# oxylusengine/Oxylus

Hardware: NVIDIA H100
Metric: meshlet_instances_culled_per_s (higher is better)
Workload: dtype f32

## Files before the change

oxylus_b200/csrc/kernels_tri.cuh:

```cuda
#pragma once
#include <climits>

#include "oxc_exact.cuh"
#include "oxc_raster_core.cuh"
#include "oxc_tma.cuh"

namespace oxc {

#ifndef OXC_TRI_THREADS
#define OXC_TRI_THREADS 256
#endif
constexpr int TRI_THREADS = OXC_TRI_THREADS;
constexpr int TRI_WARPS = TRI_THREADS / 32;

struct TriParams {
  const OxcMeshletInstance* meshlet_instances;
  const InstCull* inst;
  const InstGeom* geom;
  const OxcMeshletInstanceVisibility* vis;
  const OxcDispatchIndirectCommand* tri_cmd;
  const uint32_t* visible_indices;
  const uint32_t* id_base;
  uint32_t late;
  uint32_t* reordered_indices;
// ... 74 lines not shown
  const uint32_t id_base = p.id_base ? __ldg(p.id_base) : 0u;
  const uint32_t n_tiles = (count + TRI_WARPS - 1) / TRI_WARPS;
  float4* clip_s = clip_all[warp];
  for (uint32_t tile = blockIdx.x; tile < n_tiles; tile += gridDim.x) {
    const uint32_t g = tile * TRI_WARPS + warp;
    bool pass[2] = {false, false};
    uint32_t rank[2] = {0, 0}, wtotal = 0, data_id = 0;
    if (g < count) {
      const MeshletWork w = load_meshlet(p, first + g, id_base, clip_s, lane);
      data_id = w.data_id;
#pragma unroll
      for (int k = 0; k < 2; k++) {
        const uint32_t t = lane + 32u * k;
        float4 c0, c1, c2;
        pass[k] = t < w.tri_count && triangle_passes(w, t, clip_s, c0, c1, c2);
        if (pass[k] && p.small_primitive_cull && tri_covers_no_sample(c0, c1, c2, p.f_width, p.f_height, p.width, p.height)) pass[k] = false;
        const uint32_t bal = __ballot_sync(0xffffffffu, pass[k]);
        rank[k] = wtotal + __popc(bal & ((1u << lane) - 1u));
        wtotal += __popc(bal);
      }
      __syncwarp();
    }
    if (lane == 0) warp_cnt[warp] = wtotal;
    __syncthreads();
    if (threadIdx.x == 0) {
      uint32_t s = 0;
#pragma unroll
      for (int k = 0; k < TRI_WARPS; k++) { const uint32_t c = warp_cnt[k]; warp_cnt[k] = s; s += c; }
      base_s = s ? atomicAdd(&p.draw_cmd->index_count, s * 3u) : 0u;
    }
    __syncthreads();
    const uint32_t wbase = base_s + warp_cnt[warp] * 3u;
#pragma unroll
    for (int k = 0; k < 2; k++)
      if (pass[k]) {
        const uint32_t t = lane + 32u * k, off = wbase + rank[k] * 3u, masked = data_id << OXC_VIS_PRIMITIVE_BITS;
        p.reordered_indices[off + 0] = masked | ((t * 3u + 0u) & OXC_VIS_PRIMITIVE_MASK);
        p.reordered_indices[off + 1] = masked | ((t * 3u + 1u) & OXC_VIS_PRIMITIVE_MASK);
        p.reordered_indices[off + 2] = masked | ((t * 3u + 2u) & OXC_VIS_PRIMITIVE_MASK);
      }
    __syncthreads();
  }
}

#ifndef OXC_RASTER_MIN_BLOCKS
#define OXC_RASTER_MIN_BLOCKS 3
#endif
#ifndef OXC_RASTER_BIG_PIXELS
#define OXC_RASTER_BIG_PIXELS 32
#endif
#ifndef OXC_RASTER_BATCH
#define OXC_RASTER_BATCH 8
#endif
constexpr int MICRO_STAGE_BYTES = 224;
constexpr int RASTER_BATCH = OXC_RASTER_BATCH;
static_assert(RASTER_BATCH >= 1 && RASTER_BATCH <= 32, "one header per lane: a grab holds at most 32 meshlets");
constexpr int RASTER_BIG_PIXELS = OXC_RASTER_BIG_PIXELS;

struct MeshletHeader {
  uint32_t gid, inst, vertex_offset, vertex_count, tri_offset, tri_count;
  const uint32_t* micro;
  const uint32_t* vidx;
  const uint2* pos;
};

OXC_DI MeshletHeader fetch_header(const TriParams& p, uint32_t slot, uint32_t id_base) {
  MeshletHeader h;
  h.gid = __ldg(&p.visible_indices[slot]);
  const uint2 mi = __ldg(reinterpret_cast<const uint2*>(p.meshlet_instances) + (h.gid - id_base));
  const InstGeom* g = p.geom + mi.x;
  const uint4 g0 = __ldg(reinterpret_cast<const uint4*>(g));
  const uint4 g1 = __ldg(reinterpret_cast<const uint4*>(g) + 1);
  const OxcMeshlet* meshlets = reinterpret_cast<const OxcMeshlet*>(((uint64_t)g0.y << 32) | g0.x);
  const uint4 m = __ldg(reinterpret_cast<const uint4*>(meshlets + mi.y));
  h.inst = mi.x;
  h.vertex_offset = m.x;
  h.tri_offset = m.y;
  h.vertex_count = min(m.z, (uint32_t)OXC_MESHLET_MAX_VERTICES);
  h.tri_count = min(m.w, (uint32_t)OXC_MESHLET_MAX_PRIMITIVES);
  h.micro = reinterpret_cast<const uint32_t*>(((uint64_t)g0.w << 32) | g0.z);
  h.vidx = reinterpret_cast<const uint32_t*>(((uint64_t)g1.y << 32) | g1.x) + m.x;
  h.pos = reinterpret_cast<const uint2*>(((uint64_t)g1.w << 32) | g1.z);
  return h;
}

OXC_DI MeshletHeader bcast_header(const MeshletHeader& h, int src) {
  MeshletHeader o;
  o.gid = __shfl_sync(0xffffffffu, h.gid, src); o.inst = __shfl_sync(0xffffffffu, h.inst, src);
  o.vertex_offset = 0;
  o.vertex_count = __shfl_sync(0xffffffffu, h.vertex_count, src);
  o.tri_offset = __shfl_sync(0xffffffffu, h.tri_offset, src); o.tri_count = __shfl_sync(0xffffffffu, h.tri_count, src);
  o.micro = reinterpret_cast<const uint32_t*>(__shfl_sync(0xffffffffu, reinterpret_cast<unsigned long long>(h.micro), src));
  o.vidx = reinterpret_cast<const uint32_t*>(__shfl_sync(0xffffffffu, reinterpret_cast<unsigned long long>(h.vidx), src));
  o.pos = reinterpret_cast<const uint2*>(__shfl_sync(0xffffffffu, reinterpret_cast<unsigned long long>(h.pos), src));
  return o;
}

constexpr int BIG_CHUNK_W = 64, BIG_CHUNK_H = 32;

OXC_DI void big_entry_store(uint4* dst, const TriSetup& s, int px0, int px1, int py0, int py1, uint32_t data) {
  dst[0] = make_uint4((uint32_t)s.ax, (uint32_t)s.ay, (uint32_t)s.bx, (uint32_t)s.by);
  dst[1] = make_uint4((uint32_t)s.cx, (uint32_t)s.cy, __float_as_uint(s.za), __float_as_uint(s.dzb));
  dst[2] = make_uint4(__float_as_uint(s.dzc), (uint32_t)px0, (uint32_t)px1, (uint32_t)py0);
  dst[3] = make_uint4((uint32_t)py1, (uint32_t)s.bias, data, 0u);
}

OXC_DI void big_entry_load(const uint4* src, TriSetup& s, uint32_t& data) {
  const uint4 a = src[0], b = src[1], c = src[2], d = src[3];
  s.ax = (int)a.x; s.ay = (int)a.y; s.bx = (int)a.z; s.by = (int)a.w;
  s.cx = (int)b.x; s.cy = (int)b.y; s.za = __uint_as_float(b.z); s.dzb = __uint_as_float(b.w);
// ... 11 lines not shown
  if (base + n > p.big_capacity) {
    for (uint32_t k = base; k < p.big_capacity; k++) big_entry_store(p.big_queue + (size_t)k * 4, s, 1, 0, 1, 0, data);
    return false;
  }
  uint32_t k = base;
  for (uint32_t cy = 0; cy < ch; cy++)
    for (uint32_t cx = 0; cx < cw; cx++, k++) {
      const int x0 = s.px0 + (int)(cx * BIG_CHUNK_W), y0 = s.py0 + (int)(cy * BIG_CHUNK_H);
      big_entry_store(p.big_queue + (size_t)k * 4, s, x0, min(s.px1, x0 + BIG_CHUNK_W - 1), y0, min(s.py1, y0 + BIG_CHUNK_H - 1), data);
    }
  return true;
}

constexpr uint32_t BIG_PUSH_ALONE = 4;
OXC_DI uint32_t big_chunk_count(const TriSetup& s) {
  return ((uint32_t)(s.px1 - s.px0) / BIG_CHUNK_W + 1u) * ((uint32_t)(s.py1 - s.py0) / BIG_CHUNK_H + 1u);
}

OXC_DI bool big_push_warp(const TriParams& p, const TriSetup& s, uint32_t data, uint32_t lane) {
  const uint32_t cw = (uint32_t)(s.px1 - s.px0) / BIG_CHUNK_W + 1u, ch = (uint32_t)(s.py1 - s.py0) / BIG_CHUNK_H + 1u;
  const uint32_t n = cw * ch;
  uint32_t base = 0xFFFFFFFFu;
  if (lane == 0 && *reinterpret_cast<volatile uint32_t*>(&p.big_counters[0]) < p.big_capacity) base = atomicAdd(&p.big_counters[0], n);
  base = __shfl_sync(0xffffffffu, base, 0);
  if (base >= p.big_capacity) return false;
  if (base + n > p.big_capacity) {
    for (uint32_t k = base + lane; k < p.big_capacity; k += 32) big_entry_store(p.big_queue + (size_t)k * 4, s, 1, 0, 1, 0, data);
    return false;
  }
  for (uint32_t k = lane; k < n; k += 32) {
    const uint32_t cy = k / cw, cx = k - cy * cw;
    const int x0 = s.px0 + (int)(cx * BIG_CHUNK_W), y0 = s.py0 + (int)(cy * BIG_CHUNK_H);
    big_entry_store(p.big_queue + (size_t)(base + k) * 4, s, x0, min(s.px1, x0 + BIG_CHUNK_W - 1), y0, min(s.py1, y0 + BIG_CHUNK_H - 1), data);
  }
  return true;
}

__global__ void __launch_bounds__(256) k_raster_big(const __grid_constant__ TriParams p) {
  const uint32_t lane = threadIdx.x & 31;
  const uint32_t total = min(p.big_counters[0], p.big_capacity);
  const int lx = lane & 7, ly = lane >> 3;
  for (uint32_t i = blockIdx.x * (blockDim.x >> 5) + (threadIdx.x >> 5); i < total; i += gridDim.x * (blockDim.x >> 5)) {
    TriSetup b;
    uint32_t data;
    big_entry_load(p.big_queue + (size_t)i * 4, b, data);
    for (int ty = b.py0; ty <= b.py1; ty += 4)
      for (int tx = b.px0; tx <= b.px1; tx += 8) {
        const int px = tx + lx, py = ty + ly;
        if (px <= b.px1 && py <= b.py1) raster_pixel(b, px, py, data, p.visbuf, p.width);
      }
  }
}

template <bool PREFETCH_GRAB>
__global__ void __launch_bounds__(TRI_THREADS, OXC_RASTER_MIN_BLOCKS) k_raster_visbuffer(const __grid_constant__ TriParams p) {
  __shared__ float4 clip_all[TRI_WARPS][OXC_MESHLET_MAX_VERTICES];
  __shared__ ScreenVert scr_all[TRI_WARPS][OXC_MESHLET_MAX_VERTICES];
  const uint32_t lane = threadIdx.x & 31, warp = threadIdx.x >> 5;
#ifndef OXC_RASTER_NO_SMEM_MICRO
#define OXC_RASTER_SMEM_MICRO 1
#endif
#ifdef OXC_RASTER_SMEM_MICRO
  __shared__ uint32_t micro_w[TRI_WARPS][52];
#endif
#ifdef OXC_RASTER_TMA_MICRO
  __shared__ __align__(16) uint8_t micro_all[TRI_WARPS][MICRO_STAGE_BYTES];
  __shared__ __align__(8) uint64_t micro_bar[TRI_WARPS];
  if (lane == 0) { mbar_init(&micro_bar[warp], 1); mbar_fence_init(); }
  __syncwarp();
  uint32_t micro_phase = 0;
#endif
  const uint32_t first = p.late ? p.vis->early_visible_meshlet_instances : 0u;
  const uint32_t count = p.tri_cmd->x;
  const uint32_t id_base = p.id_base ? __ldg(p.id_base) : 0u;
  float4* clip_s = clip_all[warp];
  ScreenVert* scr_s = scr_all[warp];
  uint32_t kept = 0;
#ifdef OXC_RASTER_STATS
  unsigned long long t_entry, t_chase = 0, t_proc = 0, n_done = 0, n_grabs = 0;
  asm volatile("mov.u64 %0, %%globaltimer;" : "=l"(t_entry));
#endif
  const uint32_t n_warps2 = gridDim.x * TRI_WARPS * 2u;
  uint32_t g_next = 0, batch_next = 1;
  if (PREFETCH_GRAB && lane == 0) {
    batch_next = min((uint32_t)RASTER_BATCH, max(1u, count / n_warps2));
    g_next = atomicAdd(p.work_counter, batch_next);
  }
  for (;;) {
    uint32_t g0 = 0, batch = 1;
    if (PREFETCH_GRAB) {
      g0 = __shfl_sync(0xffffffffu, g_next, 0);
      batch = __shfl_sync(0xffffffffu, batch_next, 0);
      if (g0 >= count) break;
      if (lane == 0) {
        const uint32_t seen = g0 + batch;
        const uint32_t rem = count > seen ? count - seen : 0u;
        batch_next = min((uint32_t)RASTER_BATCH, max(1u, rem / n_warps2));
        g_next = atomicAdd(p.work_counter, batch_next);
      }
    } else {
      if (lane == 0) {
        const uint32_t seen = *reinterpret_cast<volatile uint32_t*>(p.work_counter);
        const uint32_t rem = count > seen ? count - seen : 0u;
        batch = min((uint32_t)RASTER_BATCH, max(1u, rem / n_warps2));
        g0 = atomicAdd(p.work_counter, batch);
      }
      g0 = __shfl_sync(0xffffffffu, g0, 0);
      batch = __shfl_sync(0xffffffffu, batch, 0);
      if (g0 >= count) break;
    }
    const uint32_t nb = min(batch, count - g0);
    const uint32_t my_survivor = g0 + lane;
#ifdef OXC_RASTER_STATS
    unsigned long long t_a, t_b, t_c;
    asm volatile("mov.u64 %0, %%globaltimer;" : "=l"(t_a));
#endif
    MeshletHeader mine;
    mine.gid = 0; mine.inst = 0; mine.vertex_offset = 0; mine.vertex_count = 0; mine.tri_offset = 0; mine.tri_count = 0;
    mine.micro = nullptr; mine.vidx = nullptr; mine.pos = nullptr;
    if (lane < nb) mine = fetch_header(p, first + my_survivor, id_base);
    MeshletHeader cur = bcast_header(mine, 0);
    uint32_t vi0 = lane < cur.vertex_count ? __ldg(&cur.vidx[lane]) : 0u;
    uint32_t vi1 = lane + 32u < cur.vertex_count ? __ldg(&cur.vidx[lane + 32u]) : 0u;
#ifdef OXC_RASTER_STATS
    if (vi0 + vi1 == 0xFFFFFFFFu) kept++;
    asm volatile("mov.u64 %0, %%globaltimer;" : "=l"(t_b));
#endif
    for (uint32_t j = 0; j < nb; j++) {
      const MeshletHeader w = cur;
#ifdef OXC_RASTER_TMA_MICRO
      const uint64_t micro_addr = reinterpret_cast<uint64_t>(w.micro) + w.tri_offset;
      const uint32_t micro_skew = (uint32_t)(micro_addr & 15u);
      if (lane == 0) {
        const uint32_t bytes = (micro_skew + w.tri_count * 3u + 15u) & ~15u;
        mbar_expect_tx(&micro_bar[warp], bytes);
        tma_load_1d(micro_all[warp], reinterpret_cast<const void*>(micro_addr - micro_skew), bytes, &micro_bar[warp]);
      }
#endif
#ifdef OXC_RASTER_SMEM_MICRO
      {
        const uint32_t n_words = ((w.tri_offset & 3u) + w.tri_count * 3u + 3u) >> 2;
        const uint32_t* src = w.micro + (w.tri_offset >> 2);
        const uint32_t m0 = lane < n_words ? __ldg(src + lane) : 0u;
        const uint32_t m1 = lane + 32u < n_words ? __ldg(src + lane + 32u) : 0u;
        micro_w[warp][lane] = m0;
        if (lane < 20) micro_w[warp][lane + 32] = m1;
      }
#endif
      const uint2 q0 = lane < w.vertex_count ? __ldg(&w.pos[vi0]) : make_uint2(0, 0);
      const uint2 q1 = lane + 32u < w.vertex_count ? __ldg(&w.pos[vi1]) : make_uint2(0, 0);
      if (j + 1 < nb) {
        cur = bcast_header(mine, (int)(j + 1));
        vi0 = lane < cur.vertex_count ? __ldg(&cur.vidx[lane]) : 0u;
        vi1 = lane + 32u < cur.vertex_count ? __ldg(&cur.vidx[lane + 32u]) : 0u;
      }
      const InstCull* ic = p.inst + w.inst;
      const float4 r0 = __ldg(&ic->mvp_row[0]), r1 = __ldg(&ic->mvp_row[1]), r2 = __ldg(&ic->mvp_row[2]), r3 = __ldg(&ic->mvp_row[3]);
      {
        const float x = dequantize_half_hw(q0.x & 0xFFFFu), y = dequantize_half_hw(q0.x >> 16), z = dequantize_half_hw(q0.y & 0xFFFFu);
        const float4 c = make_float4(row_dot_p1(r0, x, y, z), row_dot_p1(r1, x, y, z), row_dot_p1(r2, x, y, z), row_dot_p1(r3, x, y, z));
        clip_s[lane] = c;
        scr_s[lane] = to_screen(c, p.f_width, p.f_height);
      }
      if (w.vertex_count > 32u) {
        const float x = dequantize_half_hw(q1.x & 0xFFFFu), y = dequantize_half_hw(q1.x >> 16), z = dequantize_half_hw(q1.y & 0xFFFFu);
        const float4 c = make_float4(row_dot_p1(r0, x, y, z), row_dot_p1(r1, x, y, z), row_dot_p1(r2, x, y, z), row_dot_p1(r3, x, y, z));
        clip_s[lane + 32] = c;
        scr_s[lane + 32] = to_screen(c, p.f_width, p.f_height);
      }
      __syncwarp();
#ifdef OXC_RASTER_TMA_MICRO
      mbar_wait(&micro_bar[warp], micro_phase);
      micro_phase ^= 1u;
      const uint8_t* micro_s = micro_all[warp] + micro_skew;
#endif
      const uint32_t rounds = (w.tri_count + 31u) >> 5;
      for (uint32_t k = 0; k < rounds; k++) {
        const uint32_t t = lane + 32u * k;
        bool pass = false;
        TriSetup s;
        bool draw = false;
        if (t < w.tri_count) {
#ifdef OXC_RASTER_TMA_MICRO
          const uint32_t i0 = micro_s[t * 3u + 0u], i1 = micro_s[t * 3u + 1u], i2 = micro_s[t * 3u + 2u];
#elif defined(OXC_RASTER_SMEM_MICRO)
          const uint8_t* mb = reinterpret_cast<const uint8_t*>(micro_w[warp]) + (w.tri_offset & 3u) + t * 3u;
          const uint32_t i0 = mb[0], i1 = mb[1], i2 = mb[2];
#else
          const uint32_t base = w.tri_offset + t * 3u;
          const uint32_t i0 = micro_index(w.micro, base + 0u), i1 = micro_index(w.micro, base + 1u), i2 = micro_index(w.micro, base + 2u);
#endif
          if (max(i0, max(i1, i2)) < w.vertex_count) {
            const float4 c0 = clip_s[i0], c1 = clip_s[i1], c2 = clip_s[i2];
            pass = c0.z >= 0.0f && c1.z >= 0.0f && c2.z >= 0.0f && !triangle_backface(c0, c1, c2);
            if (pass) {
              const int why = tri_setup(scr_s[i0], scr_s[i1], scr_s[i2], p.width, p.height, s);
              draw = why == TRI_DRAW;
              if (why == TRI_NO_SAMPLE && p.small_primitive_cull) pass = false;
              if (why == TRI_INVALID_VERTEX && p.clip_queue) {
                const uint32_t slot = atomicAdd(p.clip_counter, 1u);
                if (slot < p.clip_capacity) p.clip_queue[slot] = (w.gid << p.prim_bits) | t;
                else atomicOr(p.status, (uint32_t)OXC_STATUS_CLIP_OVERFLOW);
              }
            }
          }
        }
        kept += pass ? 1u : 0u;
        const uint32_t data = (w.gid << p.prim_bits) | t;
        const int bw = draw ? s.px1 - s.px0 + 1 : 0, bh = draw ? s.py1 - s.py0 + 1 : 0;
#if defined(OXC_RASTER_STATS) && OXC_RASTER_STATS == 1
        {
          const int area = (draw && bw * bh <= RASTER_BIG_PIXELS) ? bw * bh : 0;
          const int mx = __reduce_max_sync(0xffffffffu, area), sm = __reduce_add_sync(0xffffffffu, area);
          const int nd = __popc(__ballot_sync(0xffffffffu, area > 0));
          const int nbig = __popc(__ballot_sync(0xffffffffu, draw && bw * bh > RASTER_BIG_PIXELS));
          if (lane == 0) {
            unsigned long long* st = reinterpret_cast<unsigned long long*>(p.big_queue) + (size_t)p.big_capacity * 8 + (p.late ? 64 : 0);
            atomicAdd(&st[min(mx, 33)], 1ull);
            atomicAdd(&st[40], (unsigned long long)sm);
            atomicAdd(&st[41], (unsigned long long)mx);
            atomicAdd(&st[42], (unsigned long long)nd);
            atomicAdd(&st[43], 1ull);
            atomicAdd(&st[44], (unsigned long long)nbig);
          }
        }
#endif
        bool big = draw && (bw * bh > RASTER_BIG_PIXELS);
        if (draw && !big) raster_small(s, data, p.visbuf, p.width);
        const bool few = big && big_chunk_count(s) <= BIG_PUSH_ALONE;
// ... 138 lines not shown
```

oxylus_b200/csrc/oxc_raster_core.cuh:

```cuda
#pragma once
#include <climits>

#include "oxc_exact.cuh"

namespace oxc {

struct __align__(16) ScreenVert {
  int fx, fy;
  float z;
  int pad;
};

OXC_DI ScreenVert to_screen(float4 c, float fW, float fH) {
  ScreenVert v;
  v.fx = INT_MIN; v.fy = 0; v.z = 0.f; v.pad = 0;
  if (!(c.w > 0.0f)) return v;
  const float rw = fd(1.0f, c.w);
  const float nx = fm(c.x, rw), ny = fm(c.y, rw);
  const float sx = fm(fa(fm(nx, 0.5f), 0.5f), fW), sy = fm(fa(fm(ny, 0.5f), 0.5f), fH);
  const float qx = floorf(fa(fm(sx, 256.0f), 0.5f)), qy = floorf(fa(fm(sy, 256.0f), 0.5f));
  if (!(fabsf(qx) <= 4194304.0f && fabsf(qy) <= 4194304.0f)) return v;
  v.fx = (int)qx; v.fy = (int)qy; v.z = fm(c.z, rw);
  return v;
}
// ... 31 lines not shown
  const int miny = min(v0.fy, min(v1.fy, v2.fy)), maxy = max(v0.fy, max(v1.fy, v2.fy));
  s.px0 = max(0, (minx - 128 + 255) >> 8);
  s.px1 = min((int)W - 1, (maxx - 128) >> 8);
  s.py0 = max(0, (miny - 128 + 255) >> 8);
  s.py1 = min((int)H - 1, (maxy - 128) >> 8);
  if (s.px1 < s.px0 || s.py1 < s.py0) return TRI_NO_SAMPLE;
  s.narrow = (maxx - minx) < 16384 && (maxy - miny) < 16384;
  long long area2;
  if (s.narrow) area2 = (long long)((v1.fx - v0.fx) * (v2.fy - v0.fy) - (v1.fy - v0.fy) * (v2.fx - v0.fx));
  else area2 = orient2d(v0.fx, v0.fy, v1.fx, v1.fy, v2.fx, v2.fy);
  if (area2 >= 0) return TRI_BACK_OR_DEGENERATE;
  s.ax = v0.fx; s.ay = v0.fy; s.bx = v2.fx; s.by = v2.fy; s.cx = v1.fx; s.cy = v1.fy;
  const float fa_ = (float)(-area2);
  s.za = v0.z;
  s.dzb = fd(fs(v2.z, v0.z), fa_);
  s.dzc = fd(fs(v1.z, v0.z), fa_);
  s.bias = edge_bias_bit(s.bx, s.by, s.cx, s.cy) | (edge_bias_bit(s.cx, s.cy, s.ax, s.ay) << 1) |
           (edge_bias_bit(s.ax, s.ay, s.bx, s.by) << 2);
  return TRI_DRAW;
}

OXC_DI void shade_pixel(const TriSetup& s, long long e0, long long e1, long long e2, int px, int py, uint32_t data,
                        unsigned long long* vis, uint32_t W) {
  if ((e0 - (s.bias & 1)) < 0 || (e1 - ((s.bias >> 1) & 1)) < 0 || (e2 - ((s.bias >> 2) & 1)) < 0) return;
  const float zz = fa(fa(s.za, fm((float)e1, s.dzb)), fm((float)e2, s.dzc));
  if (!(zz >= 0.0f && zz <= 1.0f)) return;
  uint32_t zb = __float_as_uint(zz);
  zb = zb == 0x80000000u ? 0u : zb;
  const unsigned long long v = ((unsigned long long)zb << 32) | data;
  unsigned long long* ptr = vis + (size_t)py * W + px;
  atomicMax(ptr, v);
}

OXC_DI void raster_pixel(const TriSetup& s, int px, int py, uint32_t data, unsigned long long* vis, uint32_t W) {
  const int sx = px * 256 + 128, sy = py * 256 + 128;
  shade_pixel(s, orient2d(s.bx, s.by, s.cx, s.cy, sx, sy), orient2d(s.cx, s.cy, s.ax, s.ay, sx, sy),
              orient2d(s.ax, s.ay, s.bx, s.by, sx, sy), px, py, data, vis, W);
}

OXC_DI int orient2d_32(int ax, int ay, int bx, int by, int cx, int cy) { return (bx - ax) * (cy - ay) - (by - ay) * (cx - ax); }

OXC_DI void shade_pixel_32(const TriSetup& s, int e0, int e1, int e2, int px, int py, uint32_t data, unsigned long long* vis,
                           uint32_t W) {
  if ((e0 - (s.bias & 1)) < 0 || (e1 - ((s.bias >> 1) & 1)) < 0 || (e2 - ((s.bias >> 2) & 1)) < 0) return;
  const float zz = fa(fa(s.za, fm((float)e1, s.dzb)), fm((float)e2, s.dzc));
  if (!(zz >= 0.0f && zz <= 1.0f)) return;
  uint32_t zb = __float_as_uint(zz);
  zb = zb == 0x80000000u ? 0u : zb;
  const unsigned long long v = ((unsigned long long)zb << 32) | data;
  unsigned long long* ptr = vis + (size_t)py * W + px;
  atomicMax(ptr, v);
}

OXC_DI void raster_small(const TriSetup& s, uint32_t data, unsigned long long* vis, uint32_t W) {
  const int sx0 = s.px0 * 256 + 128, sy0 = s.py0 * 256 + 128;
  if (s.narrow) {
    int r0 = orient2d_32(s.bx, s.by, s.cx, s.cy, sx0, sy0), r1 = orient2d_32(s.cx, s.cy, s.ax, s.ay, sx0, sy0),
        r2 = orient2d_32(s.ax, s.ay, s.bx, s.by, sx0, sy0);
    const int dx0 = -(s.cy - s.by) * 256, dy0 = (s.cx - s.bx) * 256, dx1 = -(s.ay - s.cy) * 256, dy1 = (s.ax - s.cx) * 256,
              dx2 = -(s.by - s.ay) * 256, dy2 = (s.bx - s.ax) * 256;
    for (int py = s.py0; py <= s.py1; py++) {
      int e0 = r0, e1 = r1, e2 = r2;
      for (int px = s.px0; px <= s.px1; px++) {
        shade_pixel_32(s, e0, e1, e2, px, py, data, vis, W);
        e0 += dx0; e1 += dx1; e2 += dx2;
      }
      r0 += dy0; r1 += dy1; r2 += dy2;
    }
    return;
  }
  long long r0 = orient2d(s.bx, s.by, s.cx, s.cy, sx0, sy0);
  long long r1 = orient2d(s.cx, s.cy, s.ax, s.ay, sx0, sy0);
  long long r2 = orient2d(s.ax, s.ay, s.bx, s.by, sx0, sy0);
  const long long dx0 = -(long long)(s.cy - s.by) * 256, dy0 = (long long)(s.cx - s.bx) * 256;
  const long long dx1 = -(long long)(s.ay - s.cy) * 256, dy1 = (long long)(s.ax - s.cx) * 256;
  const long long dx2 = -(long long)(s.by - s.ay) * 256, dy2 = (long long)(s.bx - s.ax) * 256;
  for (int py = s.py0; py <= s.py1; py++) {
    long long e0 = r0, e1 = r1, e2 = r2;
    for (int px = s.px0; px <= s.px1; px++) {
      shade_pixel(s, e0, e1, e2, px, py, data, vis, W);
      e0 += dx0; e1 += dx1; e2 += dx2;
    }
    r0 += dy0; r1 += dy1; r2 += dy2;
  }
}

OXC_DI float clip_plane_distance(const float4 v, int plane) {
  switch (plane) {
    case 0: return fs(v.w, v.z);
    case 1: return fa(v.w, v.x);
    case 2: return fs(v.w, v.x);
    case 3: return fa(v.w, v.y);
    default: return fs(v.w, v.y);
  }
}

OXC_DI int clip_polygon(float4 c0, float4 c1, float4 c2, float4 (*poly)[12], int& cur) {
  int n = 3;
  cur = 0;
  poly[0][0] = c0; poly[0][1] = c1; poly[0][2] = c2;
  for (int plane = 0; plane < 5 && n >= 3; plane++) {
    const float4* in = poly[cur];
    float4* out = poly[cur ^ 1];
    int m = 0;
    for (int i = 0; i < n; i++) {
      const float4 A = in[i], B = in[(i + 1) % n];
// ... 19 lines not shown
```

oxylus_b200/csrc/oxcull.cu:

```cuda
#include <cuda_runtime.h>

#include <atomic>
#include <cstdarg>
#include <cstdio>
#include <cstdlib>
#include <cstring>
#include <new>
#include <vector>

#include <dlfcn.h>
#include <nccl.h>

#include "kernels_cull.cuh"
#include "kernels_decode.cuh"
#include "kernels_hiz.cuh"
#include "kernels_mgpu.cuh"
#include "kernels_tri.cuh"
#include "kernels_alpha.cuh"

using namespace oxc;

namespace {

thread_local char g_err[512] = "";
// ... 261 lines not shown
  TRY(dalloc(&c->d_clip_queue, (size_t)c->clip_capacity));
  c->d_clip_counter = c->d_raster_work + 3;
  TRY(dalloc(&c->d_id_base_auto, 1));
  TRY(dalloc(&c->d_status, 1));
  c->prim_bits = info->wide_ids ? OXC_VIS_WIDE_PRIMITIVE_BITS : OXC_VIS_PRIMITIVE_BITS;
  if (info->alloc_reordered_indices) TRY(dalloc(&c->d_reordered, (size_t)N * OXC_MESHLET_MAX_PRIMITIVES * 3));
  if (info->max_views > 1) {
    TRY(dalloc(&c->d_view_planes, (size_t)I * info->max_views));
    TRY(dalloc(&c->d_view_bits, (size_t)N));
    TRY(dalloc(&c->d_view_counts, (size_t)OXC_MAX_VIEWS));
    TRY(dalloc(&c->d_inst_views, (size_t)I * info->max_views));
  }
  {
    uint32_t m = info->hiz_width > info->hiz_height ? info->hiz_width : info->hiz_height, levels = 0;
    while (m) { levels++; m >>= 1; }
    levels = levels < OXC_HIZ_MAX_LEVELS ? levels : OXC_HIZ_MAX_LEVELS;
    uint32_t off = 0;
    for (uint32_t l = 0; l < OXC_HIZ_MAX_LEVELS; l++) {
      c->hiz.level_offset[l] = off;
      if (l < levels) {
        uint32_t mw = info->hiz_width >> l, mh = info->hiz_height >> l;
        off += (mw < 1 ? 1 : mw) * (mh < 1 ? 1 : mh);
      }
    }
    c->hiz.width = info->hiz_width; c->hiz.height = info->hiz_height; c->hiz.levels = levels;
    c->hiz_total = off;
    TRY(dalloc(&c->d_hiz, (size_t)off));
    c->hiz.data = c->d_hiz;
  }
#undef TRY
  CK(cudaMemset(c->d_mask, 0, (size_t)c->mask_words * 4));
  CK(cudaMemset(c->d_hiz, 0, (size_t)c->hiz_total * 4));
  CK(cudaMemset(c->d_vis, 0, sizeof(OxcMeshletInstanceVisibility)));
  CK(cudaMemset(c->d_tri_counter, 0, 8));
  CK(cudaMemset(c->d_status, 0, 4));
  OxcDispatchIndirectCommand one{0, 1, 1};
  CK(cudaMemcpy(c->d_cull_meshlets_cmd, &one, sizeof one, cudaMemcpyHostToDevice));
  CK(cudaMemcpy(c->d_cull_triangles_cmd, &one, sizeof one, cudaMemcpyHostToDevice));
  OxcDrawIndexedIndirectCommand dc{0, 1, 0, 0, 0};
  CK(cudaMemcpy(c->d_draw_cmd, &dc, sizeof dc, cudaMemcpyHostToDevice));
#define OCC(dst, kern, threads) CK(cudaOccupancyMaxActiveBlocksPerMultiprocessor(&(dst), kern, threads, 0))
#define OCCC(dst, H, O, L)                                                                                                        \
  CK(cudaFuncSetAttribute(k_cull_meshlets<H, O, L, false>, cudaFuncAttributeMaxDynamicSharedMemorySize, (int)sizeof(CullShared<O && !L>)));  \
  CK(cudaFuncSetAttribute(k_cull_meshlets<H, O, L, true>, cudaFuncAttributeMaxDynamicSharedMemorySize, (int)sizeof(CullShared<O && !L>)));   \
  CK(cudaOccupancyMaxActiveBlocksPerMultiprocessor(&(dst), (k_cull_meshlets<H, O, L, false>), CULL_THREADS, sizeof(CullShared<O && !L>)))
  OCCC(c->occ_cull[0][0][0], false, false, false);
  OCCC(c->occ_cull[1][0][0], true, false, false);
  OCCC(c->occ_cull[1][0][1], true, false, true);
  OCCC(c->occ_cull[1][1][0], true, true, false);
  OCCC(c->occ_cull[1][1][1], true, true, true);
#undef OCCC
  c->occ_cull[0][0][1] = c->occ_cull[0][1][0] = c->occ_cull[0][1][1] = c->occ_cull[0][0][0];
  OCC(c->occ_tri, k_cull_triangles, TRI_THREADS);
  OCC(c->occ_raster, k_raster_visbuffer<false>, TRI_THREADS);
  OCC(c->occ_mv, k_cull_meshlets_multiview, CULL_THREADS);
#undef OCC
  *out_ctx = c;
  return OXC_OK;
}

void oxc_destroy(OxcContext* c) {
  if (!c) return;
  cudaSetDevice(c->device);
  if (c->mg.active) { cudaDeviceSynchronize(); mgpu_release(c); }
  cudaFree(c->d_meshes); cudaFree(c->d_mesh_instances); cudaFree(c->d_transforms); cudaFree(c->d_blob);
  cudaFree(c->d_lod_aabb); cudaFree(c->d_inst); cudaFree(c->d_geom); cudaFree(c->d_counts); cudaFree(c->d_block_sums);
  cudaFree(c->d_meshlet_instances); cudaFree(c->d_slabs); cudaFree(c->d_visible); cudaFree(c->d_mask); cudaFree(c->d_vis);
  cudaFree(c->d_cull_meshlets_cmd); cudaFree(c->d_cull_triangles_cmd); cudaFree(c->d_draw_cmd);
  cudaFree(c->d_reordered); cudaFree(c->d_tri_counter); cudaFree(c->d_raster_work); cudaFree(c->d_big_queue); cudaFree(c->d_clip_queue); cudaFree(c->d_id_base_auto); cudaFree(c->d_status); cudaFree(c->d_hiz);
  cudaFree(c->d_view_planes); cudaFree(c->d_view_bits); cudaFree(c->d_view_counts); cudaFree(c->d_inst_views);
  cudaFree(c->d_alpha_materials); cudaFree(c->d_alpha_lists); cudaFree(c->d_alpha_cmd);
  delete c;
}

int oxc_set_scene(OxcContext* c, const OxcSceneDesc* sc, void* stream) {
  if (!c || !sc) return fail(OXC_E_INVALID, "null argument");
  cudaStream_t s = static_cast<cudaStream_t>(stream);
  CK(cudaSetDevice(c->device));
  if (sc->mesh_instance_count > c->info.max_mesh_instances)
    return fail(OXC_E_CAPACITY, "mesh_instance_count %u > max_mesh_instances %u", sc->mesh_instance_count, c->info.max_mesh_instances);
  if (sc->mesh_count == 0 || !sc->meshes || !sc->blob || !sc->transforms || (sc->mesh_instance_count && !sc->mesh_instances))
    return fail(OXC_E_INVALID, "scene tables missing");
  struct Reloc { uint64_t lod_record, src, size; int field; };
  std::vector<Reloc> relocs;
  uint64_t reloc_bytes = 0;
  for (uint32_t m = 0; m < sc->mesh_count; m++) {
    const OxcMesh& me = sc->meshes[m];
    if (me.lod_count == 0 || me.lod_count > OXC_MESH_MAX_LODS) return fail(OXC_E_INVALID, "mesh %u: lod_count %u not in 1..%d", m, me.lod_count, OXC_MESH_MAX_LODS);
    if ((me.vertex_positions & 7u) || (me.vertex_normals & 3u) || (me.texture_coords & 3u) || (me.lods & 7u))
      return fail(OXC_E_INVALID, "mesh %u: vertex_positions / lods need 8-byte, normals / texcoords 4-byte aligned blob offsets", m);
    if (me.lods + (uint64_t)me.lod_count * sizeof(OxcMeshLOD) > sc->blob_size || me.vertex_positions + (uint64_t)me.vertex_count * 8u > sc->blob_size)
      return fail(OXC_E_INVALID, "mesh %u: offsets outside the blob", m);
    const OxcMeshLOD* lods = reinterpret_cast<const OxcMeshLOD*>(sc->blob + me.lods);
    for (uint32_t l = 0; l < me.lod_count; l++) {
      OxcMeshLOD d;
      memcpy(&d, &lods[l], sizeof d);
      if ((d.meshlets & 7u) || (d.meshlet_bounds & 7u) || (d.local_triangle_indices & 3u) || (d.indirect_vertex_indices & 3u))
        return fail(OXC_E_INVALID, "mesh %u lod %u: meshlets / meshlet_bounds need 8-byte, index arrays 4-byte aligned blob offsets", m, l);
      if (d.meshlets + (uint64_t)d.meshlet_count * sizeof(OxcMeshlet) > sc->blob_size ||
          d.meshlet_bounds + (uint64_t)d.meshlet_count * sizeof(OxcMeshletBounds) > sc->blob_size ||
          d.local_triangle_indices + (uint64_t)d.local_triangle_indices_count > sc->blob_size ||
          d.indirect_vertex_indices + (uint64_t)d.indirect_vertex_indices_count * 4u > sc->blob_size)
        return fail(OXC_E_INVALID, "mesh %u lod %u: arrays outside the blob", m, l);
      const uint64_t rec = me.lods + (uint64_t)l * sizeof(OxcMeshLOD);
      if (d.meshlets & 15u) { relocs.push_back({rec, d.meshlets, (uint64_t)d.meshlet_count * sizeof(OxcMeshlet), 0}); reloc_bytes += (relocs.back().size + 15u) & ~15ull; }
      if (d.meshlet_bounds & 15u) { relocs.push_back({rec, d.meshlet_bounds, (uint64_t)d.meshlet_count * sizeof(OxcMeshletBounds), 1}); reloc_bytes += (relocs.back().size + 15u) & ~15ull; }
    }
// ... 285 lines not shown
  uint32_t grid = (uint32_t)(c->sm_count * (c->occ_tri > 0 ? c->occ_tri : 1));
  if (grid > tiles) grid = tiles;
  if (grid == 0) grid = 1;
  k_cull_triangles<<<grid, TRI_THREADS, 0, s>>>(p);
  LAUNCHED();
  return OXC_OK;
}

int oxc_clear_visbuffer(OxcContext* c, uint64_t* vis, uint32_t w, uint32_t h, void* stream) {
  if (!c || !vis) return fail(OXC_E_INVALID, "null argument");
  cudaStream_t s = static_cast<cudaStream_t>(stream);
  CK(cudaSetDevice(c->device));
  const size_t n = (size_t)w * h;
  k_clear_visbuffer<<<c->sm_count * 8, 256, 0, s>>>(reinterpret_cast<unsigned long long*>(vis), n);
  LAUNCHED();
  CK(cudaMemsetAsync(c->d_tri_counter, 0, 8, s));
  return OXC_OK;
}

int oxc_raster_visbuffer(OxcContext* c, const OxcCullCamera* cam, uint32_t flags, uint32_t w, uint32_t h, uint64_t* vis,
                         int small_primitive_cull, void* stream) {
  if (!c || !cam || !vis) return fail(OXC_E_INVALID, "null argument");
  if (c->scene_id_bound > (1ull << (32u - c->prim_bits)))
    return fail(OXC_E_CAPACITY, "the scene can emit %llu meshlet instances: ids overflow the %u id bits of the vis-buffer word (visbuffer.slang:9-10)%s",
                (unsigned long long)c->scene_id_bound, 32u - c->prim_bits, c->info.wide_ids ? "" : "; create the context with wide_ids = 1 (26 + 6 bit packing)");
  cudaStream_t s = static_cast<cudaStream_t>(stream);
  CK(cudaSetDevice(c->device));
  TriParams p{};
  int rc = tri_common(c, cam, flags, s, &p);
  if (rc != OXC_OK) return rc;
  p.visbuf = reinterpret_cast<unsigned long long*>(vis); p.width = w; p.height = h; p.f_width = (float)w; p.f_height = (float)h;
  p.small_primitive_cull = small_primitive_cull ? 1u : 0u;
  p.work_counter = c->d_raster_work;
  CK(cudaMemsetAsync(c->d_raster_work, 0, 16, s));
  uint32_t tiles = (c->info.max_meshlet_instances + TRI_WARPS - 1) / TRI_WARPS;
  uint32_t grid = (uint32_t)(c->sm_count * (c->occ_raster > 0 ? c->occ_raster : 1));
  if (grid > tiles) grid = tiles;
  if (grid == 0) grid = 1;
  p.big_queue = c->d_big_queue; p.big_counters = c->d_big_counters; p.big_capacity = c->big_capacity;
  p.clip_queue = c->d_clip_queue; p.clip_counter = c->d_clip_counter; p.clip_capacity = c->clip_capacity;
  TriParams pm = p;
  AlphaParams ap{};
  if (c->alpha_active) {
    ap.mesh_instances = c->d_mesh_instances; ap.materials = c->d_alpha_materials; ap.material_count = c->alpha_material_count;
    ap.opaque_list = c->d_alpha_lists; ap.masked_list = c->d_alpha_lists + c->info.max_meshlet_instances;
    ap.opaque_cmd = reinterpret_cast<OxcDispatchIndirectCommand*>(c->d_alpha_cmd);
    ap.masked_cmd = reinterpret_cast<OxcDispatchIndirectCommand*>(c->d_alpha_cmd + 16);
    CK(cudaMemsetAsync(c->d_alpha_cmd, 0, 64, s));
    k_partition_alpha<<<c->sm_count * 4, 256, 0, s>>>(p, ap);
    LAUNCHED();
    pm.visible_indices = ap.opaque_list; pm.tri_cmd = ap.opaque_cmd;
    pm.vis = reinterpret_cast<const OxcMeshletInstanceVisibility*>(c->d_alpha_cmd + 32);
  }
  if (p.late) k_raster_visbuffer<true><<<grid, TRI_THREADS, 0, s>>>(pm);
  else k_raster_visbuffer<false><<<grid, TRI_THREADS, 0, s>>>(pm);
  LAUNCHED();
  k_raster_clip_queue<<<c->sm_count, 128, 0, s>>>(p);
  LAUNCHED();
  if (c->alpha_active) {
    k_raster_alpha<false><<<c->sm_count * 8, ALPHA_THREADS, 0, s>>>(p, ap);
    LAUNCHED();
  }
  k_raster_big<<<c->sm_count * 8, 256, 0, s>>>(p);
  LAUNCHED();
  return OXC_OK;
}

int oxc_raster_overdraw(OxcContext* c, const OxcCullCamera* cam, uint32_t flags, uint32_t w, uint32_t h, uint32_t* overdraw, int after_frame,
                        void* stream) {
  if (!c || !cam || !overdraw) return fail(OXC_E_INVALID, "null argument");
  cudaStream_t s = static_cast<cudaStream_t>(stream);
  CK(cudaSetDevice(c->device));
  TriParams p{};
  int rc = tri_common(c, cam, flags, s, &p);
  if (rc != OXC_OK) return rc;
  p.width = w; p.height = h; p.f_width = (float)w; p.f_height = (float)h;
  AlphaParams ap{};
  ap.mesh_instances = c->d_mesh_instances; ap.overdraw = overdraw; ap.count_from_visibility = after_frame ? 1u : 0u;
  if (c->alpha_active) { ap.materials = c->d_alpha_materials; ap.material_count = c->alpha_material_count; }
  k_raster_alpha<true><<<c->sm_count * 8, ALPHA_THREADS, 0, s>>>(p, ap);
  LAUNCHED();
  return OXC_OK;
}

int oxc_clear_overdraw(OxcContext* c, uint32_t* overdraw, uint32_t w, uint32_t h, void* stream) {
  if (!c || !overdraw) return fail(OXC_E_INVALID, "null argument");
  CK(cudaSetDevice(c->device));
  CK(cudaMemsetAsync(overdraw, 0, (size_t)w * h * 4, static_cast<cudaStream_t>(stream)));
  return OXC_OK;
}

static float host_dequantize_half(uint16_t h) {
  const uint32_t sgn = ((uint32_t)h & 0x8000u) << 16, em = (uint32_t)h & 0x7fffu;
  uint32_t r = (em + (112u << 10)) << 13;
  r = (em < (1u << 10)) ? 0u : r;
  r += (em >= (31u << 10)) ? (112u << 23) : 0u;
  const uint32_t bits = sgn | r;
  float f;
  memcpy(&f, &bits, 4);
  return f;
}

int oxc_set_materials(OxcContext* c, const OxcMaterialTable* t, void* stream) {
  if (!c) return fail(OXC_E_INVALID, "null context");
  cudaStream_t s = static_cast<cudaStream_t>(stream);
  CK(cudaSetDevice(c->device));
  if (!t || t->material_count == 0) {
    c->alpha_active = false;
// ... 678 lines not shown
```

Measured before the change: 1.807 billion.

## Always prefetch raster work grabs; add opt-in meshlet sample classification path

Drops the PREFETCH_GRAB template so every raster launch, including the early pass, issues the next atomic work grab one iteration ahead instead of reading the counter and grabbing synchronously. It also adds a compile-time CLASSIFY path, off by default. That path computes a meshlet screen bounding box with warp reductions, skips rasterizing meshlets that cover no pixel centre, and handles meshlets covering only a few samples in sample-major order with warp max reductions and a single atomicMax per pixel. The prefetch is meant to hide atomic latency in the early pass, at the cost of always holding one grab in flight.

New measurement: 2.035 billion, median of 6. +12.6%, better.

```diff
diff --git a/oxylus_b200/csrc/kernels_tri.cuh b/oxylus_b200/csrc/kernels_tri.cuh
--- a/oxylus_b200/csrc/kernels_tri.cuh
+++ b/oxylus_b200/csrc/kernels_tri.cuh
@@ -150,10 +150,21 @@
 #ifndef OXC_RASTER_BATCH
 #define OXC_RASTER_BATCH 8
 #endif
+#ifndef OXC_RASTER_CLASSIFY
+#define OXC_RASTER_CLASSIFY 0
+#endif
+#ifndef OXC_RASTER_SAMPLE_MAJOR
+#define OXC_RASTER_SAMPLE_MAJOR 4
+#endif
 constexpr int MICRO_STAGE_BYTES = 224;
 constexpr int RASTER_BATCH = OXC_RASTER_BATCH;
 static_assert(RASTER_BATCH >= 1 && RASTER_BATCH <= 32, "one header per lane: a grab holds at most 32 meshlets");
 constexpr int RASTER_BIG_PIXELS = OXC_RASTER_BIG_PIXELS;
+constexpr int RASTER_SAMPLE_MAJOR = OXC_RASTER_SAMPLE_MAJOR;
+static_assert(RASTER_SAMPLE_MAJOR >= 0 && RASTER_SAMPLE_MAJOR <= 32 && RASTER_SAMPLE_MAJOR <= RASTER_BIG_PIXELS, "sample-major limit");
+
+OXC_DI uint32_t bias_s32(int x) { return (uint32_t)x ^ 0x80000000u; }
+OXC_DI int unbias_s32(uint32_t x) { return (int)(x ^ 0x80000000u); }
 
 struct MeshletHeader {
   uint32_t gid, inst, vertex_offset, vertex_count, tri_offset, tri_count;
@@ -271,7 +282,6 @@
   }
 }
 
-template <bool PREFETCH_GRAB>
 __global__ void __launch_bounds__(TRI_THREADS, OXC_RASTER_MIN_BLOCKS) k_raster_visbuffer(const __grid_constant__ TriParams p) {
   __shared__ float4 clip_all[TRI_WARPS][OXC_MESHLET_MAX_VERTICES];
   __shared__ ScreenVert scr_all[TRI_WARPS][OXC_MESHLET_MAX_VERTICES];
@@ -301,32 +311,18 @@
 #endif
   const uint32_t n_warps2 = gridDim.x * TRI_WARPS * 2u;
   uint32_t g_next = 0, batch_next = 1;
-  if (PREFETCH_GRAB && lane == 0) {
+  if (lane == 0) {
     batch_next = min((uint32_t)RASTER_BATCH, max(1u, count / n_warps2));
     g_next = atomicAdd(p.work_counter, batch_next);
   }
   for (;;) {
-    uint32_t g0 = 0, batch = 1;
-    if (PREFETCH_GRAB) {
-      g0 = __shfl_sync(0xffffffffu, g_next, 0);
-      batch = __shfl_sync(0xffffffffu, batch_next, 0);
-      if (g0 >= count) break;
-      if (lane == 0) {
-        const uint32_t seen = g0 + batch;
-        const uint32_t rem = count > seen ? count - seen : 0u;
-        batch_next = min((uint32_t)RASTER_BATCH, max(1u, rem / n_warps2));
-        g_next = atomicAdd(p.work_counter, batch_next);
-      }
-    } else {
-      if (lane == 0) {
-        const uint32_t seen = *reinterpret_cast<volatile uint32_t*>(p.work_counter);
-        const uint32_t rem = count > seen ? count - seen : 0u;
-        batch = min((uint32_t)RASTER_BATCH, max(1u, rem / n_warps2));
-        g0 = atomicAdd(p.work_counter, batch);
-      }
-      g0 = __shfl_sync(0xffffffffu, g0, 0);
-      batch = __shfl_sync(0xffffffffu, batch, 0);
-      if (g0 >= count) break;
+    const uint32_t g0 = __shfl_sync(0xffffffffu, g_next, 0), batch = __shfl_sync(0xffffffffu, batch_next, 0);
+    if (g0 >= count) break;
+    if (lane == 0) {
+      const uint32_t seen = g0 + batch;
+      const uint32_t rem = count > seen ? count - seen : 0u;
+      batch_next = min((uint32_t)RASTER_BATCH, max(1u, rem / n_warps2));
+      g_next = atomicAdd(p.work_counter, batch_next);
     }
     const uint32_t nb = min(batch, count - g0);
     const uint32_t my_survivor = g0 + lane;
@@ -375,17 +371,35 @@
       }
       const InstCull* ic = p.inst + w.inst;
       const float4 r0 = __ldg(&ic->mvp_row[0]), r1 = __ldg(&ic->mvp_row[1]), r2 = __ldg(&ic->mvp_row[2]), r3 = __ldg(&ic->mvp_row[3]);
+#if OXC_RASTER_CLASSIFY
+      uint32_t bx0 = bias_s32(1 << 23), by0 = bias_s32(1 << 23), bx1 = bias_s32(-(1 << 23)), by1 = bias_s32(-(1 << 23));
+      bool bad = false;
+#endif
       {
         const float x = dequantize_half_hw(q0.x & 0xFFFFu), y = dequantize_half_hw(q0.x >> 16), z = dequantize_half_hw(q0.y & 0xFFFFu);
         const float4 c = make_float4(row_dot_p1(r0, x, y, z), row_dot_p1(r1, x, y, z), row_dot_p1(r2, x, y, z), row_dot_p1(r3, x, y, z));
         clip_s[lane] = c;
         scr_s[lane] = to_screen(c, p.f_width, p.f_height);
+#if OXC_RASTER_CLASSIFY
+        const ScreenVert v = scr_s[lane];
+        if (lane < w.vertex_count) {
+          bad = v.fx == INT_MIN;
+          if (!bad) { bx0 = bx1 = bias_s32(v.fx); by0 = by1 = bias_s32(v.fy); }
+        }
+#endif
       }
       if (w.vertex_count > 32u) {
         const float x = dequantize_half_hw(q1.x & 0xFFFFu), y = dequantize_half_hw(q1.x >> 16), z = dequantize_half_hw(q1.y & 0xFFFFu);
         const float4 c = make_float4(row_dot_p1(r0, x, y, z), row_dot_p1(r1, x, y, z), row_dot_p1(r2, x, y, z), row_dot_p1(r3, x, y, z));
         clip_s[lane + 32] = c;
         scr_s[lane + 32] = to_screen(c, p.f_width, p.f_height);
+#if OXC_RASTER_CLASSIFY
+        const ScreenVert v = scr_s[lane + 32];
+        if (lane + 32u < w.vertex_count) {
+          if (v.fx == INT_MIN) bad = true;
+          else { bx0 = min(bx0, bias_s32(v.fx)); bx1 = max(bx1, bias_s32(v.fx)); by0 = min(by0, bias_s32(v.fy)); by1 = max(by1, bias_s32(v.fy)); }
+        }
+#endif
       }
       __syncwarp();
 #ifdef OXC_RASTER_TMA_MICRO
@@ -394,6 +408,84 @@
       const uint8_t* micro_s = micro_all[warp] + micro_skew;
 #endif
       const uint32_t rounds = (w.tri_count + 31u) >> 5;
+#if OXC_RASTER_CLASSIFY
+      auto corners = [&](uint32_t t, uint32_t& i0, uint32_t& i1, uint32_t& i2) {
+#ifdef OXC_RASTER_TMA_MICRO
+        i0 = micro_s[t * 3u + 0u]; i1 = micro_s[t * 3u + 1u]; i2 = micro_s[t * 3u + 2u];
+#elif defined(OXC_RASTER_SMEM_MICRO)
+        const uint8_t* mb = reinterpret_cast<const uint8_t*>(micro_w[warp]) + (w.tri_offset & 3u) + t * 3u;
+        i0 = mb[0]; i1 = mb[1]; i2 = mb[2];
+#else
+        const uint32_t base = w.tri_offset + t * 3u;
+        i0 = micro_index(w.micro, base + 0u); i1 = micro_index(w.micro, base + 1u); i2 = micro_index(w.micro, base + 2u);
+#endif
+      };
+      const bool classify = w.vertex_count > 0u && !__any_sync(0xffffffffu, bad);
+      const int minx = unbias_s32(__reduce_min_sync(0xffffffffu, bx0)), maxx = unbias_s32(__reduce_max_sync(0xffffffffu, bx1));
+      const int miny = unbias_s32(__reduce_min_sync(0xffffffffu, by0)), maxy = unbias_s32(__reduce_max_sync(0xffffffffu, by1));
+      const int mpx0 = max(0, (minx - 128 + 255) >> 8), mpx1 = min((int)p.width - 1, (maxx - 128) >> 8);
+      const int mpy0 = max(0, (miny - 128 + 255) >> 8), mpy1 = min((int)p.height - 1, (maxy - 128) >> 8);
+      const int mnx = mpx1 - mpx0 + 1;
+      int samples = !classify ? INT_MAX : (mnx <= 0 || mpy1 < mpy0) ? 0 : mnx * (mpy1 - mpy0 + 1);
+      if (samples > 0 && (maxx - minx >= 16384 || maxy - miny >= 16384)) samples = INT_MAX;
+#ifdef OXC_RASTER_STATS
+      if (lane == 0)
+        atomicAdd(reinterpret_cast<unsigned long long*>(p.big_queue) + (size_t)p.big_capacity * 8 + (p.late ? 64 : 0) +
+                      (samples == 0 ? 46 : samples <= RASTER_SAMPLE_MAJOR ? 47 : 48), 1ull);
+#endif
+      if (samples == 0) {
+        if (!p.small_primitive_cull)
+          for (uint32_t t = lane; t < w.tri_count; t += 32u) {
+            uint32_t i0, i1, i2;
+            corners(t, i0, i1, i2);
+            if (max(i0, max(i1, i2)) < w.vertex_count) {
+              const float4 c0 = clip_s[i0], c1 = clip_s[i1], c2 = clip_s[i2];
+              kept += (c0.z >= 0.0f && c1.z >= 0.0f && c2.z >= 0.0f && !triangle_backface(c0, c1, c2)) ? 1u : 0u;
+            }
+          }
+        __syncwarp();
+        continue;
+      }
+      if (RASTER_SAMPLE_MAJOR > 0 && samples <= RASTER_SAMPLE_MAJOR) {
+        unsigned long long best = 0ull;
+        for (uint32_t k = 0; k < rounds; k++) {
+          const uint32_t t = lane + 32u * k;
+          bool pass = false, draw = false;
+          TriSetup s;
+          if (t < w.tri_count) {
+            uint32_t i0, i1, i2;
+            corners(t, i0, i1, i2);
+            if (max(i0, max(i1, i2)) < w.vertex_count) {
+              const float4 c0 = clip_s[i0], c1 = clip_s[i1], c2 = clip_s[i2];
+              pass = c0.z >= 0.0f && c1.z >= 0.0f && c2.z >= 0.0f && !triangle_backface(c0, c1, c2);
+              if (pass) {
+                const int why = tri_setup(scr_s[i0], scr_s[i1], scr_s[i2], p.width, p.height, s);
+                draw = why == TRI_DRAW;
+                if (why == TRI_NO_SAMPLE && p.small_primitive_cull) pass = false;
+              }
+            }
+          }
+          kept += pass ? 1u : 0u;
+          if (!__any_sync(0xffffffffu, draw)) continue;
+          const uint32_t data = (w.gid << p.prim_bits) | t;
+          int px = mpx0, py = mpy0;
+          for (uint32_t i = 0; i < (uint32_t)samples; i++) {
+            const unsigned long long f = draw ? sample_fragment_32(s, px, py, data) : 0ull;
+            const uint32_t hi = __reduce_max_sync(0xffffffffu, (uint32_t)(f >> 32));
+            const uint32_t lo = __reduce_max_sync(0xffffffffu, (uint32_t)(f >> 32) == hi ? (uint32_t)f : 0u);
+            const unsigned long long m = ((unsigned long long)hi << 32) | lo;
+            if (lane == i && m > best) best = m;
+            if (++px > mpx1) { px = mpx0; py++; }
+          }
+        }
+        if (best) {
+          const int py = mpy0 + (int)lane / mnx, px = mpx0 + (int)lane % mnx;
+          atomicMax(p.visbuf + (size_t)py * p.width + px, best);
+        }
+        __syncwarp();
+        continue;
+      }
+#endif
       for (uint32_t k = 0; k < rounds; k++) {
         const uint32_t t = lane + 32u * k;
         bool pass = false;
diff --git a/oxylus_b200/csrc/oxc_raster_core.cuh b/oxylus_b200/csrc/oxc_raster_core.cuh
--- a/oxylus_b200/csrc/oxc_raster_core.cuh
+++ b/oxylus_b200/csrc/oxc_raster_core.cuh
@@ -107,6 +107,18 @@
   atomicMax(ptr, v);
 }
 
+OXC_DI unsigned long long sample_fragment_32(const TriSetup& s, int px, int py, uint32_t data) {
+  const int sx = px * 256 + 128, sy = py * 256 + 128;
+  const int e0 = orient2d_32(s.bx, s.by, s.cx, s.cy, sx, sy), e1 = orient2d_32(s.cx, s.cy, s.ax, s.ay, sx, sy),
+            e2 = orient2d_32(s.ax, s.ay, s.bx, s.by, sx, sy);
+  if ((e0 - (s.bias & 1)) < 0 || (e1 - ((s.bias >> 1) & 1)) < 0 || (e2 - ((s.bias >> 2) & 1)) < 0) return 0ull;
+  const float zz = fa(fa(s.za, fm((float)e1, s.dzb)), fm((float)e2, s.dzc));
+  if (!(zz >= 0.0f && zz <= 1.0f)) return 0ull;
+  uint32_t zb = __float_as_uint(zz);
+  zb = zb == 0x80000000u ? 0u : zb;
+  return ((unsigned long long)zb << 32) | data;
+}
+
 OXC_DI void raster_small(const TriSetup& s, uint32_t data, unsigned long long* vis, uint32_t W) {
   const int sx0 = s.px0 * 256 + 128, sy0 = s.py0 * 256 + 128;
   if (s.narrow) {
diff --git a/oxylus_b200/csrc/oxcull.cu b/oxylus_b200/csrc/oxcull.cu
--- a/oxylus_b200/csrc/oxcull.cu
+++ b/oxylus_b200/csrc/oxcull.cu
@@ -337,7 +337,7 @@
 #undef OCCC
   c->occ_cull[0][0][1] = c->occ_cull[0][1][0] = c->occ_cull[0][1][1] = c->occ_cull[0][0][0];
   OCC(c->occ_tri, k_cull_triangles, TRI_THREADS);
-  OCC(c->occ_raster, k_raster_visbuffer<false>, TRI_THREADS);
+  OCC(c->occ_raster, k_raster_visbuffer, TRI_THREADS);
   OCC(c->occ_mv, k_cull_meshlets_multiview, CULL_THREADS);
 #undef OCC
   *out_ctx = c;
@@ -729,8 +729,7 @@
     pm.visible_indices = ap.opaque_list; pm.tri_cmd = ap.opaque_cmd;
     pm.vis = reinterpret_cast<const OxcMeshletInstanceVisibility*>(c->d_alpha_cmd + 32);
   }
-  if (p.late) k_raster_visbuffer<true><<<grid, TRI_THREADS, 0, s>>>(pm);
-  else k_raster_visbuffer<false><<<grid, TRI_THREADS, 0, s>>>(pm);
+  k_raster_visbuffer<<<grid, TRI_THREADS, 0, s>>>(pm);
   LAUNCHED();
   k_raster_clip_queue<<<c->sm_count, 128, 0, s>>>(p);
   LAUNCHED();
```
